# Jjjing2023/Distributed-Parameter-Server-for-ML-Training

Hardware: AMD Instinct MI355X
Metric: images/sec (whole node) ResNet-18 sync-PS at 1/2/4/8 MI355X; async staleness (higher is better)
Workload: dtype fp32; 1 GPU; model=resnet18-cifar (11,220,132 params, reference ResNet18(num_classes=100)), global_batch=128, per_worker_batch=128, mode=sync, sync_steps=1, codec=fp16, fetch_codec=fp32, weight_image=False, overlap=none, topology=colocated, workers=1, transport=native RCCL (psx comm), rccl_ranks=1, pair_communicators=0, hip_graph=True, deterministic=True

## Files before the change

csrc/build.py:

```python
#!/usr/bin/env python3
from __future__ import annotations

import argparse
import concurrent.futures as cf
import glob
import os
import shutil
import subprocess
import sys

HERE = os.path.dirname(os.path.abspath(__file__))
ROOT = os.path.dirname(HERE)
PKG = os.path.join(ROOT, "distributed-parameter-server-for-ml-training_amd")
OUT = os.path.join(PKG, "_native")
OBJ = os.path.join(ROOT, "build", "obj")
ARCH = os.environ.get("PSX_OFFLOAD_ARCH", "gfx950")
HIPCC = os.environ.get("HIPCC", "/opt/rocm/bin/hipcc")
CXX = os.environ.get("CXX", "g++")


def _newer(src_files, target):
    if not os.path.exists(target):
        return True
    t = os.path.getmtime(target)
    return any(os.path.getmtime(s) > t for s in src_files)


def _run(cmd):
    r = subprocess.run(cmd, stdout=subprocess.PIPE, stderr=subprocess.STDOUT, text=True)
    if r.returncode != 0:
        raise RuntimeError("command failed (%d): %s\n%s" % (r.returncode, " ".join(cmd), r.stdout))
    return r.stdout


FILE_FLAGS = {"wino_fused.hip": ["-fno-slp-vectorize"], "wino_wgrad.hip": ["-fno-slp-vectorize", "-ffp-contract=off"]}


def build(jobs: int = 8, debug: bool = False, verbose: bool = False) -> dict:
    os.makedirs(OUT, exist_ok=True)
    os.makedirs(OBJ, exist_ok=True)
    opt = ["-O1", "-g"] if debug else ["-O3"]
    k_hdrs = glob.glob(os.path.join(HERE, "kernels", "*.hpp"))
    k_srcs = sorted(glob.glob(os.path.join(HERE, "kernels", "*.hip")))
    r_hdrs = glob.glob(os.path.join(HERE, "runtime", "*.h")) + glob.glob(os.path.join(HERE, "runtime", "*.hpp"))
    r_srcs = sorted(glob.glob(os.path.join(HERE, "runtime", "*.cpp")))

    hip_flags = [f"--offload-arch={ARCH}", "-std=c++17", "-fPIC", "-Wall", "-Wno-unused-function",
                 "-Wno-unused-variable", "-munsafe-fp-atomics", "-I", os.path.join(HERE, "kernels")] + opt
    cxx_flags = ["-std=c++17", "-fPIC", "-Wall", "-pthread", "-I", os.path.join(HERE, "runtime")] + opt

    jobs_list = []
    for s in k_srcs:
        o = os.path.join(OBJ, os.path.basename(s) + ".o")
        if _newer([s] + k_hdrs, o):
            jobs_list.append([HIPCC] + hip_flags + FILE_FLAGS.get(os.path.basename(s), []) + ["-c", s, "-o", o])
    for s in r_srcs:
        o = os.path.join(OBJ, os.path.basename(s) + ".o")
        if _newer([s] + r_hdrs, o):
            jobs_list.append([CXX] + cxx_flags + ["-c", s, "-o", o])
    with cf.ThreadPoolExecutor(max_workers=max(1, jobs)) as ex:
        for out in ex.map(_run, jobs_list):
            if verbose and out.strip():
                print(out)

    libs = {}
    k_objs = [os.path.join(OBJ, os.path.basename(s) + ".o") for s in k_srcs]
    k_lib = os.path.join(OUT, "libpsx_kernels.so")
    if k_objs and _newer(k_objs, k_lib):
        _run([HIPCC, f"--offload-arch={ARCH}", "-shared", "-fPIC", "-o", k_lib] + k_objs)
    libs["kernels"] = k_lib
    r_objs = [os.path.join(OBJ, os.path.basename(s) + ".o") for s in r_srcs]
    r_lib = os.path.join(OUT, "libpsx_runtime.so")
    if r_objs and _newer(r_objs, r_lib):
        _run([CXX, "-shared", "-fPIC", "-pthread", "-o", r_lib] + r_objs + ["-lrt"])
    libs["runtime"] = r_lib

    c_srcs = sorted(glob.glob(os.path.join(HERE, "comm", "*.cpp")) + glob.glob(os.path.join(HERE, "server", "*.cpp")))
    c_hdrs = (glob.glob(os.path.join(HERE, "comm", "*.h")) + glob.glob(os.path.join(HERE, "server", "*.h")) + r_hdrs)
    c_flags = ["-std=c++17", "-fPIC", "-Wall", "-pthread", "-D__HIP_PLATFORM_AMD__", "-I", "/opt/rocm/include",
               "-I", os.path.join(HERE, "runtime"), "-I", os.path.join(HERE, "comm")] + opt
    c_objs = []
    for s in c_srcs:
        o = os.path.join(OBJ, "comm_" + os.path.basename(s) + ".o")
        c_objs.append(o)
        if _newer([s] + c_hdrs, o):
            _run([HIPCC] + c_flags + ["-c", s, "-o", o])
    c_lib = os.path.join(OUT, "libpsx_comm.so")
    if c_objs and _newer(c_objs, c_lib):
        _run([HIPCC, "-shared", "-fPIC", "-pthread", "-o", c_lib] + c_objs + ["-ldl", "-lrt"])
    libs["comm"] = c_lib

    f_src = os.path.join(HERE, "tests", "fakecomm.hip")
    f_lib = os.path.join(OUT, "testing", "libpsx_fakecomm.so")
    if os.path.exists(f_src) and _newer([f_src], f_lib):
        os.makedirs(os.path.dirname(f_lib), exist_ok=True)
        _run([HIPCC, f"--offload-arch={ARCH}", "-std=c++17", "-fPIC", "-shared", "-Wall", "-D__HIP_PLATFORM_AMD__",
              "-I", "/opt/rocm/include"] + opt + [f_src, "-o", f_lib, "-lrt", "-pthread"])
    libs["fakecomm"] = f_lib
    return libs


def build_variant(name: str, defines: list[str], jobs: int = 8) -> str:
    vout = os.path.join(OUT, "variants")
    vobj = os.path.join(OBJ, "variant_" + name)
    os.makedirs(vout, exist_ok=True)
    os.makedirs(vobj, exist_ok=True)
    k_srcs = sorted(glob.glob(os.path.join(HERE, "kernels", "*.hip")))
    flags = [f"--offload-arch={ARCH}", "-std=c++17", "-fPIC", "-O3", "-munsafe-fp-atomics", "-I",
             os.path.join(HERE, "kernels")] + [d if d.startswith("-") else f"-D{d}" for d in defines]
    cmds = [[HIPCC] + flags + FILE_FLAGS.get(os.path.basename(s_), []) +
            ["-c", s_, "-o", os.path.join(vobj, os.path.basename(s_) + ".o")] for s_ in k_srcs]
    with cf.ThreadPoolExecutor(max_workers=max(1, jobs)) as ex:
        list(ex.map(_run, cmds))
    lib = os.path.join(vout, f"libpsx_kernels_{name}.so")
    _run([HIPCC, f"--offload-arch={ARCH}", "-shared", "-fPIC", "-o", lib] +
         [os.path.join(vobj, os.path.basename(s_) + ".o") for s_ in k_srcs])
    return lib


def main(argv=None):
    ap = argparse.ArgumentParser()
    ap.add_argument("--clean", action="store_true")
    ap.add_argument("-j", type=int, default=min(8, os.cpu_count() or 1))
    ap.add_argument("--debug", action="store_true")
    ap.add_argument("-v", action="store_true")
    ap.add_argument("--variant", default=None, help="build an A/B kernel library variant (see build_variant)")
    ap.add_argument("-D", dest="defines", action="append", default=[])
    a = ap.parse_args(argv)
    if a.variant:
        print(build_variant(a.variant, a.defines, a.j))
        return 0
    if a.clean:
        shutil.rmtree(OBJ, ignore_errors=True)
        for f in glob.glob(os.path.join(OUT, "*.so")):
            os.remove(f)
    libs = build(a.j, a.debug, a.v)
    for k, v in libs.items():
        print(f"{k}: {v}")
    return 0


if __name__ == "__main__":
    sys.exit(main())
```

csrc/kernels/wino.hpp:

```cpp
#pragma once
#include "bnfin.hpp"
#include "common.hpp"

namespace psx {

PSX_DEV void wino_bt6(const float (&d)[6], float (&r)[6]) {
  r[0] = 4.f * d[0] - 5.f * d[2] + d[4];
  r[1] = -4.f * (d[1] + d[2]) + d[3] + d[4];
  r[2] = 4.f * (d[1] - d[2]) - d[3] + d[4];
  r[3] = 2.f * (d[3] - d[1]) - d[2] + d[4];
  r[4] = 2.f * (d[1] - d[3]) - d[2] + d[4];
  r[5] = 4.f * d[1] - 5.f * d[3] + d[5];
}

PSX_DEV void wino_at6(const float (&m)[6], float (&o)[4]) {
  const float a = m[1] + m[2], b = m[1] - m[2], c = m[3] + m[4], d = m[3] - m[4];
  o[0] = m[0] + a + c;
  o[1] = b + 2.f * d;
  o[2] = a + 4.f * c;
  o[3] = b + 8.f * d + m[5];
}

PSX_DEV void wino_a4(const float (&y)[4], float (&r)[6]) {
  const float e = y[0] + y[2], o = y[1] + y[3], e4 = y[0] + 4.f * y[2], o2 = 2.f * y[1] + 8.f * y[3];
  r[0] = y[0];
  r[1] = e + o;
  r[2] = e - o;
  r[3] = e4 + o2;
  r[4] = e4 - o2;
  r[5] = y[3];
}

PSX_DEV void wino_gt6(const float (&m)[6], float (&o)[3]) {
  const float a = m[1] + m[2], b = m[1] - m[2], c = m[3] + m[4], d = m[3] - m[4];
  o[0] = 0.25f * m[0] - a * (1.f / 6.f) + c * (1.f / 24.f);
  o[1] = -b * (1.f / 6.f) + d * (1.f / 12.f);
  o[2] = -a * (1.f / 6.f) + c * (1.f / 6.f) + m[5];
}

struct WinoBnFin {
  const float* gamma;
  const float* beta;
  float* run_mean;
  float* run_var;
  float* scale;
  float* shift;
  float* save_mean;
  float* save_invstd;
  unsigned* counter;
  float count, eps, momentum;
  int C;
  const float* sshift;
  float* sshift_next;
  int det;
};

struct WinoBwdStats {
  float* part;
  const float* o;
  const float* y1;
  const float* y2;
  const float* saved1;
  const float* saved2;
  int mask_store;
  const float* mask_aff;
};


PSX_DEV void wino_bwd_coef(const float* part, const BnBwdFin& f, int c, float& k1, float& k2, float& k3, double& sdz,
                           double& sxh) {
  const int C = f.C;
  sdz = slot_sum<PSX_STAT_SLOTS>(part, c, 2 * (size_t)C, f.det);
  sxh = slot_sum<PSX_STAT_SLOTS>(part, (size_t)C + c, 2 * (size_t)C, f.det);
  const float mdz = (float)(sdz / f.count), mxh = (float)(sxh / f.count);
  const float is = f.invstd[c], gm = f.gamma[c];
  k1 = gm * is;
  k2 = -gm * is * is * mxh;
  k3 = -gm * is * mdz + gm * is * is * f.mean[c] * mxh;
}

PSX_DEV float wino_bwd_apply(float dz, float y, float k1, float k2, float k3) { return fmaf(k1, dz, fmaf(k2, y, k3)); }

}
```

csrc/kernels/wino_fused.hip:

```cpp
#include "bnfin.hpp"
#include "common.hpp"
#include "wino.hpp"

#ifndef PSX_WF_PROBE
#define PSX_WF_PROBE 0
#endif
#ifndef PSX_WF_PF
#define PSX_WF_PF 0
#endif
#ifndef PSX_WF_SWZ
#define PSX_WF_SWZ 1
#endif

namespace psx {

PSX_DEV void mfma_f32_16x16x4(f32x4& acc, float a, float b) {
  acc = __builtin_amdgcn_mfma_f32_16x16x4f32(a, b, acc, 0, 0, 0);
}

constexpr int kWfT = 16;
constexpr int kWfK = 64;

struct WinoFusedArgs {
  const float* x;
  const float* U;
  float* y;
  const float* res;
  float* stats;
  float* V;
  const float* bnpart;
  const float* sshift;
  const float* ybn;
  const float* bpart;
  int H, W, C, K, T, nkb;
  int xbytes, ubytes, vbytes, ybytes;
};

template <int GG, bool RES, bool BWD, bool MAFF, bool TWO>
__global__ __launch_bounds__(512, 1) void wino_fused_kernel(WinoFusedArgs a, WinoBnFin fin, WinoBwdStats bs,
                                                            DetRed det, BnBwdFin bfin) {
  __shared__ f32x4 vb[2][4][10][64];
  __shared__ float aff[3][256];
  __shared__ float red[3][4][16];
  const int l = threadIdx.x & 63;
  const int w = __builtin_amdgcn_readfirstlane(threadIdx.x >> 6);
  const int kq = w & 3, h = w >> 2;
  const int id = xcd_remap(blockIdx.x, gridDim.x);
  const int tb = id / a.nkb, kb = id - tb * a.nkb;
  const int H = a.H, W = a.W, C = a.C, K = a.K;
  const int tw = W >> 2, tpi = (H >> 2) * tw;
  const bool bnin = a.bnpart != nullptr;
  const bool bwdin = a.bpart != nullptr;
  const float lo = bnin ? 0.f : -__builtin_inff();
  if (bwdin) {
    for (int c = threadIdx.x; c < C; c += 512) {
      float k1, k2, k3;
      double sdz, sxh;
      wino_bwd_coef(a.bpart, bfin, c, k1, k2, k3, sdz, sxh);
      aff[0][c] = k1;
      aff[1][c] = k3;
      aff[2][c] = k2;
      if (id == 0) {
        bfin.coef[c] = k1;
        bfin.coef[C + c] = k2;
        bfin.coef[2 * C + c] = k3;
        const float dg = (float)sxh * bfin.gscale, db = (float)sdz * bfin.gscale;
        if (bfin.grad_fp16) {
          reinterpret_cast<uint16_t*>(bfin.dgamma)[c] = __builtin_bit_cast(uint16_t, (_Float16)dg);
          reinterpret_cast<uint16_t*>(bfin.dbeta)[c] = __builtin_bit_cast(uint16_t, (_Float16)db);
        } else {
          reinterpret_cast<float*>(bfin.dgamma)[c] = dg;
          reinterpret_cast<float*>(bfin.dbeta)[c] = db;
        }
      }
    }
  } else if (!bnin) {
    for (int c = threadIdx.x; c < C; c += 512) {
      aff[0][c] = 1.f;
      aff[1][c] = 0.f;
    }
  } else {
    for (int c = threadIdx.x; c < C; c += 512) {
      const double s = slot_sum<PSX_STAT_SLOTS>(a.bnpart, c, 2 * (size_t)C, fin.det);
      const double ss = slot_sum<PSX_STAT_SLOTS>(a.bnpart, (size_t)C + c, 2 * (size_t)C, fin.det);
      double mean, var;
      bn_moments(s, ss, fin.count, fin.sshift ? fin.sshift[c] : 0.f, mean, var);
      const float invstd = (float)(1.0 / sqrt(var + (double)fin.eps));
      const float sc = fin.gamma[c] * invstd, sh = fin.beta[c] - (float)mean * sc;
      aff[0][c] = sc;
      aff[1][c] = sh;
      if (id == 0) {
        fin.scale[c] = sc;
        fin.shift[c] = sh;
        fin.save_mean[c] = (float)mean;
        fin.save_invstd[c] = invstd;
        if (fin.sshift_next) fin.sshift_next[c] = (float)mean;
        if (fin.run_mean) {
          const double unb = fin.count > 1.f ? var * fin.count / (fin.count - 1.0) : var;
          fin.run_mean[c] = (1.f - fin.momentum) * fin.run_mean[c] + fin.momentum * (float)mean;
          fin.run_var[c] = (1.f - fin.momentum) * fin.run_var[c] + fin.momentum * (float)unb;
        }
      }
    }
  }
  __syncthreads();

  const int tl = 4 * kq + (l >> 4), cl = l & 15;
  const int t = tb * kWfT + tl;
  const int la = (cl & 3) * 16 + tl, qa = cl >> 2;
  int rowoff[6], coloff[6];
  unsigned okr = 0, okc = 0;
  {
    const int n = t / tpi, rem = t - n * tpi, ti = rem / tw, tj = rem - ti * tw;
#pragma unroll
    for (int r = 0; r < 6; ++r) {
      const int hh = 4 * ti - 1 + r, wc = 4 * tj - 1 + r;
      const bool oh = (unsigned)hh < (unsigned)H, ow = (unsigned)wc < (unsigned)W;
      okr |= (unsigned)oh << r;
      okc |= (unsigned)ow << r;
      rowoff[r] = (((n * H + (oh ? hh : (hh < 0 ? 0 : H - 1))) * W) * C + cl) * 4;
      coloff[r] = (ow ? wc : (wc < 0 ? 0 : W - 1)) * C * 4;
    }
  }
  const auto xr = __builtin_amdgcn_make_buffer_rsrc(const_cast<float*>(a.x), 0, a.xbytes, 0x00020000);
  const auto ybr = __builtin_amdgcn_make_buffer_rsrc(const_cast<float*>(a.ybn), 0, bwdin ? a.xbytes : 0, 0x00020000);
  const auto ur = __builtin_amdgcn_make_buffer_rsrc(const_cast<float*>(a.U), 0, a.ubytes, 0x00020000);
  const int S4 = C >> 2;
  const int ubase = ((kb * 4 + kq) * S4 * 10 + h * 5) * 1024;
  constexpr int G = GG;
  const auto vr = __builtin_amdgcn_make_buffer_rsrc(a.V, 0, a.V ? a.vbytes : 0, 0x00020000);
  const auto vnull = __builtin_amdgcn_make_buffer_rsrc(a.V, 0, 0, 0x00020000);
  const int voff = (t * C + cl) * 4;

  auto swz = [](int q, int u) { return PSX_WF_SWZ ? (u ^ ((((u >> 4) << 2) + q) & 15)) : u; };
  float d[36], yb[36];
  auto load_patch = [&](int g) {
    const int so = g * 16 * 4;
#pragma unroll
    for (int r = 0; r < 6; ++r)
#pragma unroll
      for (int s = 0; s < 6; ++s)
        d[r * 6 + s] = (PSX_WF_PROBE & 2) ? (float)(rowoff[r] + coloff[s] + so)
                                          : __uint_as_float(__builtin_amdgcn_raw_buffer_load_b32(xr, rowoff[r] + coloff[s], so, 0));
    if (bwdin) {
#pragma unroll
      for (int r = 0; r < 6; ++r)
#pragma unroll
        for (int s = 0; s < 6; ++s)
          yb[r * 6 + s] = __uint_as_float(__builtin_amdgcn_raw_buffer_load_b32(ybr, rowoff[r] + coloff[s], so, 0));
    }
  };
  auto xform = [&](int g, int p, bool real) {
    if constexpr ((PSX_WF_PROBE & 32) != 0) return;
    const int ch0 = g * 16;
    const float sc = aff[0][ch0 + cl], sh = aff[1][ch0 + cl];
    float e[36];
    if (bwdin) {
      const float k2 = aff[2][ch0 + cl];
#pragma unroll
      for (int r = 0; r < 6; ++r)
#pragma unroll
        for (int s = 0; s < 6; ++s) d[r * 6 + s] = wino_bwd_apply(d[r * 6 + s], yb[r * 6 + s], sc, k2, sh);
    }
#pragma unroll
    for (int r = 0; r < 6; ++r)
#pragma unroll
      for (int s = 0; s < 6; ++s) {
        const float v = bwdin ? d[r * 6 + s] : fmaxf(d[r * 6 + s] * sc + sh, lo);
        e[r * 6 + s] = ((okr >> r) & (okc >> s) & 1u) ? v : 0.f;
      }
#pragma unroll
    for (int s = 0; s < 6; ++s) {
      float col[6] = {e[s], e[6 + s], e[12 + s], e[18 + s], e[24 + s], e[30 + s]}, o[6];
      wino_bt6(col, o);
#pragma unroll
      for (int r = 0; r < 6; ++r) e[r * 6 + s] = o[r];
    }
#pragma unroll
    for (int r = 0; r < 6; ++r) {
      float row[6] = {e[r * 6], e[r * 6 + 1], e[r * 6 + 2], e[r * 6 + 3], e[r * 6 + 4], e[r * 6 + 5]}, o[6];
      wino_bt6(row, o);
#pragma unroll
      for (int s = 0; s < 6; ++s) e[r * 6 + s] = o[s];
    }
#pragma unroll
    for (int hh = 0; hh < 2; ++hh) {
#pragma unroll
      for (int i = 0; i < 4; ++i) {
        const int b = 18 * hh + 4 * i;
        vb[p][qa][5 * hh + i][swz(qa, la)] = (f32x4){e[b], e[b + 1], e[b + 2], e[b + 3]};
      }
      vb[p][qa][5 * hh + 4][swz(qa, la)] = (f32x4){e[18 * hh + 16], e[18 * hh + 17], 0.f, 0.f};
    }
    const auto rs = (real && kb == 0) ? vr : vnull;
    if ((PSX_WF_PROBE & 8) == 0 && a.V)
#pragma unroll
    for (int b = 0; b < 36; ++b)
      __builtin_amdgcn_raw_buffer_store_b32(__float_as_uint(e[b]), rs, voff, (b * a.T * C + ch0) * 4, 0);
  };

  f32x4 acc[18];
#pragma unroll
  for (int m = 0; m < 18; ++m) acc[m] = (f32x4){0.f, 0.f, 0.f, 0.f};
  constexpr int UD = (PSX_WF_PF & 1) ? 2 : 1;
  f32x4 ub[UD][4];
  float2 uh[UD];
  auto load_u = [&](int s, int slot) {
    const int so = ubase + s * 10 * 1024;
    if constexpr ((PSX_WF_PROBE & 1) != 0) {
#pragma unroll
      for (int i = 0; i < 4; ++i) ub[slot][i] = (f32x4){(float)so, 1.f, 2.f, (float)i};
      uh[slot] = make_float2((float)so, 1.f);
      return;
    }
#pragma unroll
    for (int i = 0; i < 4; ++i)
      ub[slot][i] = __builtin_bit_cast(f32x4, __builtin_amdgcn_raw_buffer_load_b128(ur, l * 16 + i * 1024, so, 0));
    uh[slot] = __builtin_bit_cast(float2, __builtin_amdgcn_raw_buffer_load_b64(ur, l * 16 + 4 * 1024, so, 0));
  };
#pragma unroll
  for (int i = 0; i < UD; ++i) load_u(i < S4 ? i : S4 - 1, i);
  if (h == 0) {
    load_patch(0);
    xform(0, 0, true);
    load_patch(G > 1 ? 1 : 0);
  }
  __syncthreads();
  f32x4 an[4];
  float2 ah;
  auto load_a = [&](int p, int q) {
    if constexpr ((PSX_WF_PROBE & 16) != 0) {
#pragma unroll
      for (int i = 0; i < 4; ++i) an[i] = (f32x4){(float)p, (float)q, (float)i, 1.f};
      ah = make_float2((float)q, 2.f);
      return;
    }
#pragma unroll
    for (int i = 0; i < 4; ++i) an[i] = vb[p][q][5 * h + i][swz(q, l)];
    ah = *reinterpret_cast<const float2*>(&vb[p][q][5 * h + 4][swz(q, l)]);
  };
#pragma unroll
  for (int g = 0; g < G; ++g) {
    const int p = g & 1;
    if (h == 0) {
      xform(g + 1, p ^ 1, g + 1 < G);
      load_patch(g + 2 < G ? g + 2 : G - 1);
    }
    if constexpr ((PSX_WF_PF & 2) != 0) load_a(p, 0);
#pragma unroll
    for (int q = 0; q < 4; ++q) {
      const int s = g * 4 + q;
      if constexpr ((PSX_WF_PF & 2) == 0) load_a(p, q);
      const f32x4 a0 = an[0], a1 = an[1], a2 = an[2], a3 = an[3];
      const float2 a4 = ah;
      if constexpr ((PSX_WF_PF & 2) != 0)
        if (q < 3) load_a(p, q + 1);
      const int us = s % UD;
      const f32x4 u0 = ub[us][0], u1 = ub[us][1], u2 = ub[us][2], u3 = ub[us][3];
      const float2 u4 = uh[us];
      load_u(s + UD < S4 ? s + UD : S4 - 1, us);
#pragma unroll
      for (int j = 0; j < 4; ++j) {
        mfma_f32_16x16x4(acc[j], a0[j], u0[j]);
        mfma_f32_16x16x4(acc[4 + j], a1[j], u1[j]);
        mfma_f32_16x16x4(acc[8 + j], a2[j], u2[j]);
        mfma_f32_16x16x4(acc[12 + j], a3[j], u3[j]);
      }
      mfma_f32_16x16x4(acc[16], a4.x, u4.x);
      mfma_f32_16x16x4(acc[17], a4.y, u4.y);
    }
    __syncthreads();
  }

  float at[4][3];
  {
    const float c0[4][3] = {{1.f, 1.f, 1.f}, {0.f, 1.f, -1.f}, {0.f, 1.f, 1.f}, {0.f, 1.f, -1.f}};
    const float c1[4][3] = {{1.f, 1.f, 0.f}, {2.f, -2.f, 0.f}, {4.f, 4.f, 0.f}, {8.f, -8.f, 1.f}};
#pragma unroll
    for (int r = 0; r < 4; ++r)
#pragma unroll
      for (int rr = 0; rr < 3; ++rr) at[r][rr] = h ? c1[r][rr] : c0[r][rr];
  }
  float yp[4][16];
#pragma unroll
  for (int i = 0; i < 4; ++i) {
    float z[3][4];
#pragma unroll
    for (int rr = 0; rr < 3; ++rr) {
      float row[6] = {acc[6 * rr][i], acc[6 * rr + 1][i], acc[6 * rr + 2][i],
                      acc[6 * rr + 3][i], acc[6 * rr + 4][i], acc[6 * rr + 5][i]};
      wino_at6(row, z[rr]);
    }
#pragma unroll
    for (int r = 0; r < 4; ++r)
#pragma unroll
      for (int j = 0; j < 4; ++j) yp[i][r * 4 + j] = at[r][0] * z[0][j] + at[r][1] * z[1][j] + at[r][2] * z[2][j];
  }
  float* xb = reinterpret_cast<float*>(&vb[0][0][0][0]);
  float* mine = xb + ((size_t)(kq * 2 + h) * 64 + l) * 36;
  const float* theirs = xb + ((size_t)(kq * 2 + (1 - h)) * 64 + l) * 36;
  float yv[2][16];
  if (h) {
#pragma unroll
    for (int e = 0; e < 32; e += 4)
      *reinterpret_cast<f32x4*>(mine + e) =
          (f32x4){yp[e >> 4][e & 15], yp[e >> 4][(e & 15) + 1], yp[e >> 4][(e & 15) + 2], yp[e >> 4][(e & 15) + 3]};
#pragma unroll
    for (int ii = 0; ii < 2; ++ii)
#pragma unroll
      for (int e = 0; e < 16; ++e) yv[ii][e] = yp[2 + ii][e];
  } else {
#pragma unroll
    for (int e = 0; e < 32; e += 4)
      *reinterpret_cast<f32x4*>(mine + e) = (f32x4){yp[2 + (e >> 4)][e & 15], yp[2 + (e >> 4)][(e & 15) + 1],
                                                    yp[2 + (e >> 4)][(e & 15) + 2], yp[2 + (e >> 4)][(e & 15) + 3]};
#pragma unroll
    for (int ii = 0; ii < 2; ++ii)
#pragma unroll
      for (int e = 0; e < 16; ++e) yv[ii][e] = yp[ii][e];
  }
  __syncthreads();
#pragma unroll
  for (int e = 0; e < 32; e += 4) {
    const f32x4 t4 = *reinterpret_cast<const f32x4*>(theirs + e);
#pragma unroll
    for (int j = 0; j < 4; ++j) yv[e >> 4][(e & 15) + j] += t4[j];
  }

  const int k = kb * kWfK + kq * 16 + (l & 15);
  constexpr bool bwd = BWD, two = BWD && TWO;
  float m1 = 0.f, i1 = 0.f, m2 = 0.f, i2 = 0.f, msc = 0.f, msh = 0.f;
  if constexpr (bwd) {
    m1 = bs.saved1[k];
    i1 = bs.saved1[K + k];
    if constexpr (MAFF) {
      msc = bs.mask_aff[k];
      msh = bs.mask_aff[K + k];
    }
    if constexpr (two) {
      m2 = bs.saved2[k];
      i2 = bs.saved2[K + k];
    }
  }
  const float kshift = (!bwd && a.sshift) ? a.sshift[k] : 0.f;
  const int ybytes = a.ybytes;
  const auto yr = __builtin_amdgcn_make_buffer_rsrc(a.y, 0, ybytes, 0x00020000);
#ifdef PSX_WF_RES_BUF
  const auto rr_ = __builtin_amdgcn_make_buffer_rsrc(const_cast<float*>(a.res), 0, RES ? ybytes : 0, 0x00020000);
#endif
  const auto y1r = __builtin_amdgcn_make_buffer_rsrc(const_cast<float*>(bs.y1), 0, bwd ? ybytes : 0, 0x00020000);
  const auto orr = __builtin_amdgcn_make_buffer_rsrc(const_cast<float*>(bs.o), 0, (bwd && !MAFF) ? ybytes : 0,
                                                     0x00020000);
  const auto y2r = __builtin_amdgcn_make_buffer_rsrc(const_cast<float*>(bs.y2), 0, two ? ybytes : 0, 0x00020000);
  const bool mstore = bwd && bs.mask_store;
  float s1 = 0.f, s2 = 0.f, s3 = 0.f;
#pragma unroll
  for (int ii = 0; ii < 2; ++ii) {
    const int tt = tb * kWfT + 4 * (l >> 4) + 2 * h + ii;
    const int n = tt / tpi, rem = tt - n * tpi, ti = rem / tw, tj = rem - ti * tw;
    const int base = ((((n * H + 4 * ti) * W + 4 * tj) * K) + k) * 4;
    float rv[16], y1v[16], ov[16], y2v[16];
#pragma unroll
    for (int e = 0; e < 16; ++e) {
      const int so = ((e >> 2) * W + (e & 3)) * K * 4;
#ifdef PSX_WF_RES_BUF
      if constexpr (RES) rv[e] = __uint_as_float(__builtin_amdgcn_raw_buffer_load_b32(rr_, base, so, 0));
#else
      if constexpr (RES) rv[e] = a.res[(base + so) >> 2];
#endif
      if constexpr (bwd) {
        y1v[e] = __uint_as_float(__builtin_amdgcn_raw_buffer_load_b32(y1r, base, so, 0));
        if constexpr (!MAFF) ov[e] = __uint_as_float(__builtin_amdgcn_raw_buffer_load_b32(orr, base, so, 0));
        if constexpr (two) y2v[e] = __uint_as_float(__builtin_amdgcn_raw_buffer_load_b32(y2r, base, so, 0));
      }
    }
#pragma unroll
    for (int e = 0; e < 16; ++e) {
      const int so = ((e >> 2) * W + (e & 3)) * K * 4;
      float v = yv[ii][e];
      if constexpr (RES) v += rv[e];
      if constexpr (bwd) {
        const float y1 = y1v[e];
        bool pos;
        if constexpr (MAFF)
          pos = y1 * msc + msh > 0.f;
        else
          pos = ov[e] > 0.f;
        const float dz = pos ? v : 0.f;
        s1 += dz;
        s2 += dz * (y1 - m1) * i1;
        if constexpr (two) s3 += dz * (y2v[e] - m2) * i2;
        __builtin_amdgcn_raw_buffer_store_b32(__float_as_uint(mstore ? dz : v), yr, base, so, 0);
      } else {
        __builtin_amdgcn_raw_buffer_store_b32(__float_as_uint(v), yr, base, so, 0);
        const float dd = v - kshift;
        s1 += dd;
        s2 += dd * dd;
      }
    }
  }
  float* dst = bwd ? bs.part : a.stats;
  if (!dst) return;
  const int nst = bwd ? (two ? 3 : 2) : 2;
  s1 += __shfl_xor(s1, 16, 64);
  s1 += __shfl_xor(s1, 32, 64);
  s2 += __shfl_xor(s2, 16, 64);
  s2 += __shfl_xor(s2, 32, 64);
  if constexpr (two) {
    s3 += __shfl_xor(s3, 16, 64);
    s3 += __shfl_xor(s3, 32, 64);
  }
  if (h == 1 && l < 16) {
    red[0][kq][l] = s1;
    red[1][kq][l] = s2;
    red[2][kq][l] = s3;
  }
  __syncthreads();
  float* row = dst + (size_t)(tb & (PSX_STAT_SLOTS - 1)) * nst * K;
  if (h == 0 && l < 16) {
    stat_add(det, row, k, s1 + red[0][kq][l]);
    stat_add(det, row, K + k, s2 + red[1][kq][l]);
    if constexpr (two) stat_add(det, row, 2 * K + k, s3 + red[2][kq][l]);
  }
}

}

using namespace psx;

extern "C" {

int psx_wino_fused_ok(int N, int H, int W, int C, int K) {
  if (H % 4 || W % 4 || (C != 64 && C != 128) || K % kWfK) return 0;
  const long T = (long)N * (H / 4) * (W / 4);
  return T % kWfT == 0 && (long)N * H * W * (long)(C > K ? C : K) * 4 < (1L << 31) && 40L * C * K * 4 < (1L << 31) &&
         36L * T * C < (1L << 31);
}

int psx_wino_fused(const float* x, const float* Uf, float* y, const float* res, float* stats, float* V, int N, int H,
                   int W, int C, int K, const WinoBwdStats* bst, const float* bnpart, const WinoBnFin* bnfin,
                   const float* sshift, const float* ybn, const float* bpart, const BnBwdFin* bbfin,
                   hipStream_t st) {
  if (!psx_wino_fused_ok(N, H, W, C, K)) return -2;
  if (bnpart && (!bnfin || bnfin->C != C)) return -3;
  if (bpart && (!bbfin || bbfin->C != C || !ybn || bnpart)) return -3;
  const int T = N * (H / 4) * (W / 4);
  WinoFusedArgs a{x, Uf, y, res, bst ? nullptr : stats, V, bnpart, sshift, bpart ? ybn : nullptr, bpart, H, W, C, K, T,
                  K / kWfK,
                  (int)((long)N * H * W * C * 4), (int)(40L * C * K * 4), (int)(36L * T * C * 4),
                  (int)((long)N * H * W * K * 4)};
  WinoBnFin bf{};
  if (bnpart) bf = *bnfin;
  bf.det = (int)det_enabled();
  WinoBwdStats bs{};
  if (bst) bs = *bst;
  const int rows = T / kWfT;
  DetRed det{};
  if (bst || stats) det = det_for(bst ? bst->part : stats);
  using FK = void (*)(WinoFusedArgs, WinoBnFin, WinoBwdStats, DetRed, BnBwdFin);
  BnBwdFin bb{};
  if (bpart) bb = *bbfin;
  bb.det = (int)det_enabled();
#define PSX_WF_ROW(G, R)                                                                                     \
  {wino_fused_kernel<G, R, false, false, false>, wino_fused_kernel<G, R, true, false, false>,                 \
   wino_fused_kernel<G, R, true, false, true>, wino_fused_kernel<G, R, true, true, false>,                    \
   wino_fused_kernel<G, R, true, true, true>}
  static const FK kF[2][2][5] = {{PSX_WF_ROW(4, false), PSX_WF_ROW(4, true)}, {PSX_WF_ROW(8, false), PSX_WF_ROW(8, true)}};
#undef PSX_WF_ROW
  const int var = bst ? 1 + 2 * (bs.mask_aff != nullptr) + (bs.y2 != nullptr) : 0;
  hipLaunchKernelGGL(kF[C == 128][res != nullptr][var], dim3((unsigned)(rows * (K / kWfK))), dim3(512), 0, st, a, bf, bs, det, bb);
  return (int)hipGetLastError();
}

}
```

Baseline: 39580 images/s.

## Specialize fused Winograd kernel on input mode and V store, prefetch epilogue loads

Adds template parameters for the input-affine mode (plain, BN-in, backward-in) and for whether the V tensor is stored, so the plain path skips the affine table fill, one barrier, the per-element affine/ReLU, and dead V stores, and the last group no longer does a dummy transform. The input mask becomes bitwise AND with sign-extended bit masks. Input-transform arithmetic is rewritten with explicit FMAs and contraction turned off to keep a fixed rounding order. Residual and backward epilogue loads are issued during the last group of the main loop to hide their latency, at the cost of more live registers in a kernel launched with launch bounds of 512 threads and 1 block.

```diff
diff --git a/csrc/build.py b/csrc/build.py
--- a/csrc/build.py
+++ b/csrc/build.py
@@ -36,6 +36,12 @@
 FILE_FLAGS = {"wino_fused.hip": ["-fno-slp-vectorize"], "wino_wgrad.hip": ["-fno-slp-vectorize", "-ffp-contract=off"]}
 
 
+def kernel_flags(opt, src=None) -> list:
+    flags = [f"--offload-arch={ARCH}", "-std=c++17", "-fPIC", "-Wall", "-Wno-unused-function",
+             "-Wno-unused-variable", "-munsafe-fp-atomics", "-I", os.path.join(HERE, "kernels")] + list(opt)
+    return flags + (FILE_FLAGS.get(os.path.basename(src), []) if src else [])
+
+
 def build(jobs: int = 8, debug: bool = False, verbose: bool = False) -> dict:
     os.makedirs(OUT, exist_ok=True)
     os.makedirs(OBJ, exist_ok=True)
@@ -45,8 +51,7 @@
     r_hdrs = glob.glob(os.path.join(HERE, "runtime", "*.h")) + glob.glob(os.path.join(HERE, "runtime", "*.hpp"))
     r_srcs = sorted(glob.glob(os.path.join(HERE, "runtime", "*.cpp")))
 
-    hip_flags = [f"--offload-arch={ARCH}", "-std=c++17", "-fPIC", "-Wall", "-Wno-unused-function",
-                 "-Wno-unused-variable", "-munsafe-fp-atomics", "-I", os.path.join(HERE, "kernels")] + opt
+    hip_flags = kernel_flags(opt)
     cxx_flags = ["-std=c++17", "-fPIC", "-Wall", "-pthread", "-I", os.path.join(HERE, "runtime")] + opt
 
     jobs_list = []
diff --git a/csrc/kernels/wino.hpp b/csrc/kernels/wino.hpp
--- a/csrc/kernels/wino.hpp
+++ b/csrc/kernels/wino.hpp
@@ -11,6 +11,17 @@
   r[3] = 2.f * (d[3] - d[1]) - d[2] + d[4];
   r[4] = 2.f * (d[1] - d[3]) - d[2] + d[4];
   r[5] = 4.f * d[1] - 5.f * d[3] + d[5];
+}
+
+template <bool COL>
+PSX_DEV void wino_bt6_fused(const float (&d)[6], float (&r)[6]) {
+#pragma clang fp contract(off)
+  r[0] = (COL ? __builtin_fmaf(-5.f, d[2], 4.f * d[0]) : __builtin_fmaf(4.f, d[0], -5.f * d[2])) + d[4];
+  r[1] = __builtin_fmaf(-4.f, d[1] + d[2], d[3]) + d[4];
+  r[2] = __builtin_fmaf(4.f, d[1] - d[2], -d[3]) + d[4];
+  r[3] = __builtin_fmaf(2.f, d[3] - d[1], -d[2]) + d[4];
+  r[4] = __builtin_fmaf(2.f, d[1] - d[3], -d[2]) + d[4];
+  r[5] = __builtin_fmaf(4.f, d[1], -5.f * d[3]) + d[5];
 }
 
 PSX_DEV void wino_at6(const float (&m)[6], float (&o)[4]) {
diff --git a/csrc/kernels/wino_fused.hip b/csrc/kernels/wino_fused.hip
--- a/csrc/kernels/wino_fused.hip
+++ b/csrc/kernels/wino_fused.hip
@@ -10,6 +10,9 @@
 #endif
 #ifndef PSX_WF_SWZ
 #define PSX_WF_SWZ 1
+#endif
+#ifndef PSX_WF_EARLY
+#define PSX_WF_EARLY 1
 #endif
 
 namespace psx {
@@ -36,7 +39,9 @@
   int xbytes, ubytes, vbytes, ybytes;
 };
 
-template <int GG, bool RES, bool BWD, bool MAFF, bool TWO>
+constexpr int kWfPlain = 0, kWfBnIn = 1, kWfBwdIn = 2;
+
+template <int GG, bool RES, bool BWD, bool MAFF, bool TWO, int IN, bool HASV>
 __global__ __launch_bounds__(512, 1) void wino_fused_kernel(WinoFusedArgs a, WinoBnFin fin, WinoBwdStats bs,
                                                             DetRed det, BnBwdFin bfin) {
   __shared__ f32x4 vb[2][4][10][64];
@@ -49,10 +54,9 @@
   const int tb = id / a.nkb, kb = id - tb * a.nkb;
   const int H = a.H, W = a.W, C = a.C, K = a.K;
   const int tw = W >> 2, tpi = (H >> 2) * tw;
-  const bool bnin = a.bnpart != nullptr;
-  const bool bwdin = a.bpart != nullptr;
-  const float lo = bnin ? 0.f : -__builtin_inff();
-  if (bwdin) {
+  constexpr bool bnin = IN == kWfBnIn;
+  const bool bwdin = IN == kWfBwdIn && a.bpart != nullptr;
+  if constexpr (IN == kWfBwdIn) {
     for (int c = threadIdx.x; c < C; c += 512) {
       float k1, k2, k3;
       double sdz, sxh;
@@ -74,12 +78,7 @@
         }
       }
     }
-  } else if (!bnin) {
-    for (int c = threadIdx.x; c < C; c += 512) {
-      aff[0][c] = 1.f;
-      aff[1][c] = 0.f;
-    }
-  } else {
+  } else if constexpr (bnin) {
     for (int c = threadIdx.x; c < C; c += 512) {
       const double s = slot_sum<PSX_STAT_SLOTS>(a.bnpart, c, 2 * (size_t)C, fin.det);
       const double ss = slot_sum<PSX_STAT_SLOTS>(a.bnpart, (size_t)C + c, 2 * (size_t)C, fin.det);
@@ -103,7 +102,7 @@
       }
     }
   }
-  __syncthreads();
+  if constexpr (IN != kWfPlain) __syncthreads();
 
   const int tl = 4 * kq + (l >> 4), cl = l & 15;
   const int t = tb * kWfT + tl;
@@ -128,8 +127,7 @@
   const int S4 = C >> 2;
   const int ubase = ((kb * 4 + kq) * S4 * 10 + h * 5) * 1024;
   constexpr int G = GG;
-  const auto vr = __builtin_amdgcn_make_buffer_rsrc(a.V, 0, a.V ? a.vbytes : 0, 0x00020000);
-  const auto vnull = __builtin_amdgcn_make_buffer_rsrc(a.V, 0, 0, 0x00020000);
+  const auto vr = __builtin_amdgcn_make_buffer_rsrc(a.V, 0, (HASV && kb == 0) ? a.vbytes : 0, 0x00020000);
   const int voff = (t * C + cl) * 4;
 
   auto swz = [](int q, int u) { return PSX_WF_SWZ ? (u ^ ((((u >> 4) << 2) + q) & 15)) : u; };
@@ -150,10 +148,14 @@
           yb[r * 6 + s] = __uint_as_float(__builtin_amdgcn_raw_buffer_load_b32(ybr, rowoff[r] + coloff[s], so, 0));
     }
   };
-  auto xform = [&](int g, int p, bool real) {
+  auto xform = [&](int g, int p) {
     if constexpr ((PSX_WF_PROBE & 32) != 0) return;
     const int ch0 = g * 16;
-    const float sc = aff[0][ch0 + cl], sh = aff[1][ch0 + cl];
+    float sc = 1.f, sh = 0.f;
+    if constexpr (IN != kWfPlain) {
+      sc = aff[0][ch0 + cl];
+      sh = aff[1][ch0 + cl];
+    }
     float e[36];
     if (bwdin) {
       const float k2 = aff[2][ch0 + cl];
@@ -162,24 +164,35 @@
 #pragma unroll
         for (int s = 0; s < 6; ++s) d[r * 6 + s] = wino_bwd_apply(d[r * 6 + s], yb[r * 6 + s], sc, k2, sh);
     }
+    unsigned mr[6], mc[6];
+#pragma unroll
+    for (int r = 0; r < 6 && IN != kWfBwdIn; ++r) {
+      mr[r] = (unsigned)__builtin_amdgcn_sbfe((int)okr, r, 1);
+      mc[r] = (unsigned)__builtin_amdgcn_sbfe((int)okc, r, 1);
+      asm("" : "+v"(mr[r]));
+      asm("" : "+v"(mc[r]));
+    }
 #pragma unroll
     for (int r = 0; r < 6; ++r)
 #pragma unroll
       for (int s = 0; s < 6; ++s) {
-        const float v = bwdin ? d[r * 6 + s] : fmaxf(d[r * 6 + s] * sc + sh, lo);
-        e[r * 6 + s] = ((okr >> r) & (okc >> s) & 1u) ? v : 0.f;
+        const float v = bnin ? fmaxf(d[r * 6 + s] * sc + sh, 0.f) : d[r * 6 + s];
+        if constexpr (IN != kWfBwdIn)
+          e[r * 6 + s] = __uint_as_float(__float_as_uint(v) & mr[r] & mc[s]);
+        else
+          e[r * 6 + s] = ((okr >> r) & (okc >> s) & 1u) ? v : 0.f;
       }
 #pragma unroll
     for (int s = 0; s < 6; ++s) {
       float col[6] = {e[s], e[6 + s], e[12 + s], e[18 + s], e[24 + s], e[30 + s]}, o[6];
-      wino_bt6(col, o);
+      wino_bt6_fused<true>(col, o);
 #pragma unroll
       for (int r = 0; r < 6; ++r) e[r * 6 + s] = o[r];
     }
 #pragma unroll
     for (int r = 0; r < 6; ++r) {
       float row[6] = {e[r * 6], e[r * 6 + 1], e[r * 6 + 2], e[r * 6 + 3], e[r * 6 + 4], e[r * 6 + 5]}, o[6];
-      wino_bt6(row, o);
+      wino_bt6_fused<false>(row, o);
 #pragma unroll
       for (int s = 0; s < 6; ++s) e[r * 6 + s] = o[s];
     }
@@ -192,11 +205,11 @@
       }
       vb[p][qa][5 * hh + 4][swz(qa, la)] = (f32x4){e[18 * hh + 16], e[18 * hh + 17], 0.f, 0.f};
     }
-    const auto rs = (real && kb == 0) ? vr : vnull;
-    if ((PSX_WF_PROBE & 8) == 0 && a.V)
-#pragma unroll
-    for (int b = 0; b < 36; ++b)
-      __builtin_amdgcn_raw_buffer_store_b32(__float_as_uint(e[b]), rs, voff, (b * a.T * C + ch0) * 4, 0);
+    if constexpr (HASV && (PSX_WF_PROBE & 8) == 0) {
+#pragma unroll
+      for (int b = 0; b < 36; ++b)
+        __builtin_amdgcn_raw_buffer_store_b32(__float_as_uint(e[b]), vr, voff, (b * a.T * C + ch0) * 4, 0);
+    }
   };
 
   f32x4 acc[18];
@@ -222,8 +235,8 @@
   for (int i = 0; i < UD; ++i) load_u(i < S4 ? i : S4 - 1, i);
   if (h == 0) {
     load_patch(0);
-    xform(0, 0, true);
-    load_patch(G > 1 ? 1 : 0);
+    xform(0, 0);
+    if constexpr (G > 1) load_patch(1);
   }
   __syncthreads();
   f32x4 an[4];
@@ -239,12 +252,51 @@
     for (int i = 0; i < 4; ++i) an[i] = vb[p][q][5 * h + i][swz(q, l)];
     ah = *reinterpret_cast<const float2*>(&vb[p][q][5 * h + 4][swz(q, l)]);
   };
+  const int k = kb * kWfK + kq * 16 + (l & 15);
+  constexpr bool bwd = BWD, two = BWD && TWO;
+  const int ybytes = a.ybytes;
+#ifdef PSX_WF_RES_BUF
+  const auto rr_ = __builtin_amdgcn_make_buffer_rsrc(const_cast<float*>(a.res), 0, RES ? ybytes : 0, 0x00020000);
+#endif
+  const auto y1r = __builtin_amdgcn_make_buffer_rsrc(const_cast<float*>(bs.y1), 0, bwd ? ybytes : 0, 0x00020000);
+  const auto orr = __builtin_amdgcn_make_buffer_rsrc(const_cast<float*>(bs.o), 0, (bwd && !MAFF) ? ybytes : 0,
+                                                     0x00020000);
+  const auto y2r = __builtin_amdgcn_make_buffer_rsrc(const_cast<float*>(bs.y2), 0, two ? ybytes : 0, 0x00020000);
+  float rv[2][16], y1v[2][16], ov[2][16], y2v[2][16];
+  auto out_base = [&](int ii) {
+    const int tt = tb * kWfT + 4 * (l >> 4) + 2 * h + ii;
+    const int n = tt / tpi, rem = tt - n * tpi, ti = rem / tw, tj = rem - ti * tw;
+    return ((((n * H + 4 * ti) * W + 4 * tj) * K) + k) * 4;
+  };
+  auto load_epi = [&](int ii) {
+    const int base = out_base(ii);
+#pragma unroll
+    for (int e = 0; e < 16; ++e) {
+      const int so = ((e >> 2) * W + (e & 3)) * K * 4;
+#ifdef PSX_WF_RES_BUF
+      if constexpr (RES) rv[ii][e] = __uint_as_float(__builtin_amdgcn_raw_buffer_load_b32(rr_, base, so, 0));
+#else
+      if constexpr (RES) rv[ii][e] = a.res[(base + so) >> 2];
+#endif
+      if constexpr (bwd) {
+        y1v[ii][e] = __uint_as_float(__builtin_amdgcn_raw_buffer_load_b32(y1r, base, so, 0));
+        if constexpr (!MAFF) ov[ii][e] = __uint_as_float(__builtin_amdgcn_raw_buffer_load_b32(orr, base, so, 0));
+        if constexpr (two) y2v[ii][e] = __uint_as_float(__builtin_amdgcn_raw_buffer_load_b32(y2r, base, so, 0));
+      }
+    }
+  };
+  constexpr bool early = PSX_WF_EARLY && (RES || BWD);
 #pragma unroll
   for (int g = 0; g < G; ++g) {
     const int p = g & 1;
+    if constexpr (early)
+      if (g == G - 1) {
+        load_epi(0);
+        if constexpr (PSX_WF_EARLY > 1) load_epi(1);
+      }
     if (h == 0) {
-      xform(g + 1, p ^ 1, g + 1 < G);
-      load_patch(g + 2 < G ? g + 2 : G - 1);
+      if (g + 1 < G) xform(g + 1, p ^ 1);
+      if (g + 2 < G) load_patch(g + 2);
     }
     if constexpr ((PSX_WF_PF & 2) != 0) load_a(p, 0);
 #pragma unroll
@@ -327,8 +379,6 @@
     for (int j = 0; j < 4; ++j) yv[e >> 4][(e & 15) + j] += t4[j];
   }
 
-  const int k = kb * kWfK + kq * 16 + (l & 15);
-  constexpr bool bwd = BWD, two = BWD && TWO;
   float m1 = 0.f, i1 = 0.f, m2 = 0.f, i2 = 0.f, msc = 0.f, msh = 0.f;
   if constexpr (bwd) {
     m1 = bs.saved1[k];
@@ -343,53 +393,29 @@
     }
   }
   const float kshift = (!bwd && a.sshift) ? a.sshift[k] : 0.f;
-  const int ybytes = a.ybytes;
   const auto yr = __builtin_amdgcn_make_buffer_rsrc(a.y, 0, ybytes, 0x00020000);
-#ifdef PSX_WF_RES_BUF
-  const auto rr_ = __builtin_amdgcn_make_buffer_rsrc(const_cast<float*>(a.res), 0, RES ? ybytes : 0, 0x00020000);
-#endif
-  const auto y1r = __builtin_amdgcn_make_buffer_rsrc(const_cast<float*>(bs.y1), 0, bwd ? ybytes : 0, 0x00020000);
-  const auto orr = __builtin_amdgcn_make_buffer_rsrc(const_cast<float*>(bs.o), 0, (bwd && !MAFF) ? ybytes : 0,
-                                                     0x00020000);
-  const auto y2r = __builtin_amdgcn_make_buffer_rsrc(const_cast<float*>(bs.y2), 0, two ? ybytes : 0, 0x00020000);
   const bool mstore = bwd && bs.mask_store;
   float s1 = 0.f, s2 = 0.f, s3 = 0.f;
 #pragma unroll
   for (int ii = 0; ii < 2; ++ii) {
-    const int tt = tb * kWfT + 4 * (l >> 4) + 2 * h + ii;
-    const int n = tt / tpi, rem = tt - n * tpi, ti = rem / tw, tj = rem - ti * tw;
-    const int base = ((((n * H + 4 * ti) * W + 4 * tj) * K) + k) * 4;
-    float rv[16], y1v[16], ov[16], y2v[16];
-#pragma unroll
-    for (int e = 0; e < 16; ++e) {
-      const int so = ((e >> 2) * W + (e & 3)) * K * 4;
-#ifdef PSX_WF_RES_BUF
-      if constexpr (RES) rv[e] = __uint_as_float(__builtin_amdgcn_raw_buffer_load_b32(rr_, base, so, 0));
-#else
-      if constexpr (RES) rv[e] = a.res[(base + so) >> 2];
-#endif
-      if constexpr (bwd) {
-        y1v[e] = __uint_as_float(__builtin_amdgcn_raw_buffer_load_b32(y1r, base, so, 0));
-        if constexpr (!MAFF) ov[e] = __uint_as_float(__builtin_amdgcn_raw_buffer_load_b32(orr, base, so, 0));
-        if constexpr (two) y2v[e] = __uint_as_float(__builtin_amdgcn_raw_buffer_load_b32(y2r, base, so, 0));
-      }
-    }
+    const int base = out_base(ii);
+    if (!(early && (ii == 0 || PSX_WF_EARLY > 1))) load_epi(ii);
 #pragma unroll
     for (int e = 0; e < 16; ++e) {
       const int so = ((e >> 2) * W + (e & 3)) * K * 4;
       float v = yv[ii][e];
-      if constexpr (RES) v += rv[e];
+      if constexpr (RES) v += rv[ii][e];
       if constexpr (bwd) {
-        const float y1 = y1v[e];
+        const float y1 = y1v[ii][e];
         bool pos;
         if constexpr (MAFF)
           pos = y1 * msc + msh > 0.f;
         else
-          pos = ov[e] > 0.f;
+          pos = ov[ii][e] > 0.f;
         const float dz = pos ? v : 0.f;
         s1 += dz;
         s2 += dz * (y1 - m1) * i1;
-        if constexpr (two) s3 += dz * (y2v[e] - m2) * i2;
+        if constexpr (two) s3 += dz * (y2v[ii][e] - m2) * i2;
         __builtin_amdgcn_raw_buffer_store_b32(__float_as_uint(mstore ? dz : v), yr, base, so, 0);
       } else {
         __builtin_amdgcn_raw_buffer_store_b32(__float_as_uint(v), yr, base, so, 0);
@@ -461,14 +487,29 @@
   BnBwdFin bb{};
   if (bpart) bb = *bbfin;
   bb.det = (int)det_enabled();
-#define PSX_WF_ROW(G, R)                                                                                     \
-  {wino_fused_kernel<G, R, false, false, false>, wino_fused_kernel<G, R, true, false, false>,                 \
-   wino_fused_kernel<G, R, true, false, true>, wino_fused_kernel<G, R, true, true, false>,                    \
-   wino_fused_kernel<G, R, true, true, true>}
-  static const FK kF[2][2][5] = {{PSX_WF_ROW(4, false), PSX_WF_ROW(4, true)}, {PSX_WF_ROW(8, false), PSX_WF_ROW(8, true)}};
-#undef PSX_WF_ROW
-  const int var = bst ? 1 + 2 * (bs.mask_aff != nullptr) + (bs.y2 != nullptr) : 0;
-  hipLaunchKernelGGL(kF[C == 128][res != nullptr][var], dim3((unsigned)(rows * (K / kWfK))), dim3(512), 0, st, a, bf, bs, det, bb);
+#define PSX_WF_F(G, R, I, V) wino_fused_kernel<G, R, false, false, false, I, V>
+#define PSX_WF_FROW(G, R)                                                                        \
+  {{PSX_WF_F(G, R, kWfPlain, false), PSX_WF_F(G, R, kWfPlain, true)},                            \
+   {PSX_WF_F(G, R, kWfBnIn, false), PSX_WF_F(G, R, kWfBnIn, true)},                              \
+   {PSX_WF_F(G, R, kWfBwdIn, false), nullptr}}
+#define PSX_WF_B(G, R, M, T) {wino_fused_kernel<G, R, true, M, T, kWfPlain, false>, wino_fused_kernel<G, R, true, M, T, kWfBwdIn, false>}
+#define PSX_WF_BROW(G, R) {PSX_WF_B(G, R, false, false), PSX_WF_B(G, R, false, true), PSX_WF_B(G, R, true, false), PSX_WF_B(G, R, true, true)}
+  static const FK kFwd[2][2][3][2] = {{PSX_WF_FROW(4, false), PSX_WF_FROW(4, true)}, {PSX_WF_FROW(8, false), PSX_WF_FROW(8, true)}};
+  static const FK kBwd[2][2][4][2] = {{PSX_WF_BROW(4, false), PSX_WF_BROW(4, true)}, {PSX_WF_BROW(8, false), PSX_WF_BROW(8, true)}};
+#undef PSX_WF_F
+#undef PSX_WF_FROW
+#undef PSX_WF_B
+#undef PSX_WF_BROW
+  const int in = bpart ? kWfBwdIn : bnpart ? kWfBnIn : kWfPlain;
+  FK fk;
+  if (bst) {
+    if (in == kWfBnIn || V) return -3;
+    fk = kBwd[C == 128][res != nullptr][2 * (bs.mask_aff != nullptr) + (bs.y2 != nullptr)][in == kWfBwdIn];
+  } else {
+    fk = kFwd[C == 128][res != nullptr][in][V != nullptr];
+    if (!fk) return -3;
+  }
+  hipLaunchKernelGGL(fk, dim3((unsigned)(rows * (K / kWfK))), dim3(512), 0, st, a, bf, bs, det, bb);
   return (int)hipGetLastError();
 }
 
```

Result: faster. 40870 images/s (median of 6 runs) (+3.3%).
